# flo-stilz/Audio-Key-Estimation

Measured on AMD Instinct MI355X. Metric: clips/s (15 s @ 22.05 kHz), HIP CQT + PitchClassNet forward, higher is better.
Workload: dtype f32 accumulation everywhere; pitch / semitone / layer-0 convolutions: f16 activations x f16 weights (per-channel power-of-two scaled) on MFMA, one product; last layer's pitch-class convolutions and heads: 3-term split-bf16 on MFMA (hi*hi + lo*hi + hi*lo); CQT filter bank: 3-term split-bf16 on MFMA

## Files before the change

audio-key-estimation_amd/csrc/pcnet_forward.h:

```cpp
#pragma once

namespace {

struct Fwd {
    const ake_pcnet* n;
    Buffers& b;
    hipStream_t s;
    bool train;
    const Route& r;

    float* p2pin_up(int i) const { return train ? b.aff_p2pin[i] + 3 * n->dims[i].prev_p : nullptr; }
    double* stats_of(int bn) const { return b.stats + 2 * n->bns[bn].ch_off; }
    int stats_stride() const { return 2 * n->bn_channels; }

    int finalize_bn(int bn, double count, float* aff_out, float slope = kSlope) {
        const auto& l = n->bns[bn];
        return ake::launch("bn_finalize_kernel", bn_finalize_kernel, dim3((l.C + 63) / 64), dim3(64), 0, s, stats_of(bn), stats_stride(),
                           count, n->blob_dev + l.gamma_off, n->blob_dev + l.beta_off, aff_out, b.bstats + 3 * l.ch_off, l.C, slope);
    }
    int identity(float* aff, int C) {
        return ake::launch_untimed("affine_identity_kernel", affine_identity_kernel, dim3((C + 63) / 64), dim3(64), 0, s, aff, C);
    }

    int conv(const ConvSite& cs, int kind, Src src, const float* in_aff, int B, int H, int T_in, bool same, float* dst, int ctot, int coff,
// ... 368 lines not shown
                    else if (g.in == P2pIn::SrcF16x4)
                        io.src = Src{reinterpret_cast<const float*>(b.melh + static_cast<size_t>(c0) * P * Ti), 1,
                                     reinterpret_cast<const float*>(reinterpret_cast<const uint2*>(b.psix[1]) + static_cast<size_t>(c0) * 36 * Ti), d.prev_pc, 36};
                    else io.src = sdesc;
                    switch (g.out) {
                        case P2pOut::Plane: io.plane = reinterpret_cast<unsigned short*>(out.p); break;
                        case P2pOut::Nchw: io.dst = out.p; break;
                        case P2pOut::Semi: io.dst = out.p; io.semi = &n->semi[i].eval; break;
                        case P2pOut::SemiFold: io.dst = cat; io.dst_ctot = ctot; io.fold_coff = d.prev_pc; io.semi = &n->semi[i].eval; break;
                    }
                    if (last_conv) last_out = g.out;
                    AKE_REQUIRE(g.ok || g.in == P2pIn::Planes || g.in == P2pIn::Src, AKE_ERR_STATE,
                                "pcnet: the route promised an input form only the persistent pitch conv reads, for a chunk (%d clips) it does not take", B);
                    if (g.ok) rc = run_p2p_f16_ps(n, n->p2p[i][j].eval, g, io, B, P, Ti, s, "conv_p2p_f16_kernel");
                    else rc = run_p2p_f16(n, n->p2p[i][j].eval, io.planes, j == 0 ? &io.src : nullptr, B, P, Ti, io.dst, d.out_p, io.plane, s, "conv_p2p_f16_kernel");
                    if (rc) return rc;
                }
            } else if ((rc = stack(0, i, sdesc, in_aff, B, P, Ti, "conv_mfma_kernel/p2p", &out, rp.x3_convs, rk.x3))) return rc;
            if (last_out == P2pOut::SemiFold) {
            } else if (last_out == P2pOut::Semi) {
                if ((rc = run_fold_max("fold_max_kernel", out.p, nullptr, d.out_p, P / 3, B, Ti, cat, ctot, d.prev_pc, s))) return rc;
            } else if (c.stay_sixth && train) {
                if ((rc = run_fold_max("fold_affine_kernel", out.p, out.aff, d.out_p, P, B, Ti, cat, ctot, d.prev_pc, s))) return rc;
                if ((rc = identity(b.aff_cat[i] + 3 * d.prev_pc, d.out_p))) return rc;
            } else if (c.stay_sixth) {
                if ((rc = fold_maps(i, out.p, d.out_p, P, B, Ti, cat, ctot, d.prev_pc))) return rc;
            } else if ((rc = semi(i, out.p, out.aff, B, P, Ti, cat, ctot, d.prev_pc, train ? b.aff_cat[i] + 3 * d.prev_pc : nullptr))) return rc;
            if (last) return AKE_OK;
            Slot pdst;
            if ((rc = stack(1, i, Src{cat, ctot, nullptr, 0, 0}, b.cat_slot(train, i).aff, B, 12, Ti, "conv_mfma_kernel/pc2pc", &pdst))) return rc;
            float* catn = b.cat_at(i + 1, c0);
            if ((rc = time_pool(pdst.p, pdst.aff, B, d.out_pc, 12, Ti, catn, b.cat_ch(i + 1), 0))) return rc;
            if (train && (rc = identity(b.aff_cat[i + 1], d.out_pc))) return rc;
            if ((rc = time_pool(out.p, out.aff, B, d.out_p, P, Ti, b.ppool[i], d.out_p, 0))) return rc;
            pc_cur = catn; p_cur = b.ppool[i]; cp = d.out_p;
        }
        return AKE_OK;
    }

    int last_pc_stack(int B, Slot* feat) {
        const auto& c = n->cfg;
        const int L = c.num_layers, i = L - 1, Ti = b.Tl[i];
        const Slot src = L == 1 ? Slot{b.fold0, nullptr} : b.cat_slot(train, i);
        const int cin = L == 1 ? 1 : n->dims[i].prev_pc + n->dims[i].out_p;
        const char* const label = L == 1 ? "conv_mfma_kernel/pc2pc0" : "conv_mfma_kernel/pc2pc";
        int rc;
        *feat = Slot{b.pcf, nullptr};
        if (r.pc == PcStack::Fused)
            return run_pc2pc_fused(n, i, src.p, cin, B, Ti, b.pcf, r.heads != HeadForm::Generic ? b.feat_cl : nullptr, s);
        Slot out;
        if (r.pc == PcStack::Bf16) {
            const unsigned short* in = reinterpret_cast<const unsigned short*>(b.pcb[i]);
            if ((rc = run_nchw_to_cl16(src.p, cin, B, Ti, reinterpret_cast<unsigned short*>(b.pcb[i]), s))) return rc;
            for (int j = 0; j < c.conv_layers; ++j) {
                const bool last_conv = j == c.conv_layers - 1;
                out = b.pc_out(false, i, j);
                if ((rc = run_pc_bf16(n, n->pc2pc[i][j].eval, in, B, Ti, true, true, last_conv ? out.p : nullptr,
                                      last_conv ? nullptr : reinterpret_cast<unsigned short*>(out.p), s, "conv_pc_bf16_kernel/pc2pc")))
                    return rc;
                in = reinterpret_cast<const unsigned short*>(out.p);
            }
        } else if (c.denseblock) {
            if ((rc = dense_stack(i, 1, src.p, n->final_ch, cin, B, 12, Ti, b.pca[i], label))) return rc;
            out = Slot{src.p, nullptr};
        } else if ((rc = stack(1, i, Src{src.p, cin, nullptr, 0, 0}, src.aff, B, 12, Ti, label, &out, r.pc_x3_convs))) return rc;
        if (L == 1) { *feat = out; return AKE_OK; }
        return time_pool(out.p, out.aff, B, n->final_ch, 12, Ti, b.pcf, n->final_ch, 0);
    }

    int heads_fused(int B, const PoolArgs& pool, float* const outs[3], int* Tm, int* pooled) {
        const int nh = r.genre_bf ? 3 : 2, Tf = b.Tf;
        float* const maps[3] = {b.map_k, b.map_t, b.map_g};
        HeadsFusedArgs ha;
        std::memset(&ha, 0, sizeof(ha));
        ha.xh = b.feat_cl; ha.xl = b.feat_cl + static_cast<long long>(B) * 12 * Tf * 16;
        for (int h = 0; h < nh; ++h) {
            const PackedConv& p0 = n->heads[h].convs[0].eval;
            const PackedConv& p1 = n->heads[h].convs[1].eval;
            ha.bfragA[h] = n->bf_frags_dev + p0.bf_off; ha.biasA[h] = n->blob_dev + p0.b_off; ha.KHA[h] = p0.kh;
            ha.bfragB[h] = n->bf_frags_dev + p1.bf_off; ha.biasB[h] = n->blob_dev + p1.b_off; ha.KHB[h] = p1.kh;
            ha.dst[h] = maps[h];
            ha.pout[h] = outs[h];
        }
        if (r.genre_bf) { ha.hs[0] = 2; ha.hs[1] = 0; ha.hs[2] = 1; }
        else { ha.hs[0] = 0; ha.hs[1] = 1; ha.hs[2] = 1; }
        ha.batch = B; ha.T_in = Tf; ha.T1 = r.T1; ha.T2 = r.T2; ha.TpA = r.T1 + 8; ha.TpB = r.TpB; ha.JB = (r.T2 + 15) / 16;
        ha.fin_off = static_cast<int>(r.hf_lds / sizeof(float)) - 12 * r.T2;
        ha.pool = pool;
        *Tm = r.T2; *pooled = nh;
        static ake::DeviceOnce hf_attr;
        const int rc = ake::raise_lds_limit(hf_attr, 150 * 1024, heads_fused_kernel<3>, heads_fused_kernel<4>);
        if (rc) return rc;
        return r.heads_mt == 3 ? ake::launch("heads_fused_kernel", heads_fused_kernel<3>, dim3(nh * B), dim3(512), r.hf_lds, s, ha)
                               : ake::launch("heads_fused_kernel", heads_fused_kernel<4>, dim3(nh * B), dim3(512), r.hf_lds, s, ha);
    }

    int heads_head1(int B, const PoolArgs& pool, float* const outs[3], int* Tm, int* pooled) {
        const int nh = r.genre_bf ? 3 : 2, Tf = b.Tf, T1 = r.T1, T2 = r.T2;
        const Head* const heads = n->heads;
        float* const maps[3] = {b.map_k, b.map_t, b.map_g};
        Head1BfArgs ha;
        std::memset(&ha, 0, sizeof(ha));
        int rc;
        for (int h = 0; h < nh; ++h) {
            const PackedConv& p0 = heads[h].convs[0].eval;
            const PackedConv& p1 = heads[h].convs[1].eval;
            unsigned short* planes = reinterpret_cast<unsigned short*>(b.head_out(false, h, 0, false).p);
            if (h == 0) {
                PcBf16Opts tonic;
                tonic.pc2 = &heads[1].convs[0].eval; tonic.planes_out2 = reinterpret_cast<unsigned short*>(b.head_out(false, 1, 0, false).p);
                if ((rc = run_pc_bf16(n, p0, b.feat_cl, B, Tf, false, true, nullptr, planes, s, "conv_pc_bf16_kernel/head", tonic))) return rc;
            }
            if (h == 2 && (rc = run_pc_bf16(n, p0, b.feat_cl, B, Tf, false, true, nullptr, planes, s, "conv_pc_bf16_kernel/genre_head")))
                return rc;
            ha.xh[h] = planes; ha.xl[h] = planes + static_cast<long long>(B) * 12 * T1 * 32;
            ha.bfrag[h] = n->bf_frags_dev + p1.bf_off; ha.bias[h] = n->blob_dev + p1.b_off; ha.dst[h] = maps[h];
            ha.KH[h] = p1.kh; ha.circular[h] = p1.kh == 12 ? 1 : 0; ha.H_out[h] = ha.circular[h] ? 12 : 12 - p1.kh + 1;
        }
        ha.T_in = T1; ha.T_out = T2; ha.JB = (T2 + 15) / 16; ha.Tp = r.TpB;
        size_t lds = std::max(static_cast<size_t>(2) * 12 * ha.Tp * 4 * sizeof(uint4), static_cast<size_t>(8) * kHead1MT * 4 * 64 * sizeof(float));
        if (r.heads_pool) {
            ha.fin_off = static_cast<int>(lds / sizeof(float));
            lds += static_cast<size_t>(12) * T2 * sizeof(float);
            for (int h = 0; h < nh; ++h) ha.pout[h] = outs[h];
            ha.pool = pool;
        }
        *Tm = T2; *pooled = r.heads_pool ? nh : 0;
        static ake::DeviceOnce h1_attr;
        if ((rc = ake::raise_lds_limit(h1_attr, 150 * 1024, conv_head1_bf16_kernel))) return rc;
        AKE_REQUIRE(lds <= 150 * 1024, AKE_ERR_UNSUPPORTED, "heads: %d frames do not fit conv_head1_bf16_kernel", T1);
        return ake::launch("conv_head1_bf16_kernel", conv_head1_bf16_kernel, dim3(B, nh), dim3(512), lds, s, ha);
    }

    int heads_generic(int first, Slot feat, int B, int* Tm) {
        const auto& c = n->cfg;
        const Head* const heads = n->heads;
        const int Tf = b.Tf;
        bool head_planes_ready = false;
        int rc;
        for (int h = first; h < (c.genre ? 3 : 2); ++h) {
            for (int j = 0; j < c.head_layers; ++j) {
                const ConvSite& cs = heads[h].convs[j];
                const PackedConv& pe = cs.eval;
                const bool lastj = j == c.head_layers - 1;
                const Slot src = j == 0 ? feat : b.head_out(train, h, j - 1, false);
                const int hc = j == 0 ? n->final_ch : heads[h].convs[j - 1].eval.cout, Tcur = Tf - j * (c.kernel_size - 1);
                const Slot dst = b.head_out(train, h, j, lastj);
                if (r.heads != HeadForm::Generic && h < 2 && j == 0) {
                    if ((rc = run_pc_bf16(n, pe, b.feat_cl, B, Tcur, false, true, dst.p, nullptr, s, "conv_pc_bf16_kernel/head"))) return rc;
                    continue;
                }
                if (train && j == 0 && !lastj && pc_f16x3_ok(cs.train, Tcur, false)) {
                    if (!head_planes_ready) {
                        if ((rc = run_nchw_to_cl16_f16x2(src.p, hc, B, Tcur, src.aff, b.feat_cl, s))) return rc;
                        head_planes_ready = true;
                    }
                    if ((rc = pc_x3_train(cs, b.feat_cl, B, Tcur, false, heads[h].kind == 2 ? 12 - cs.train.kh + 1 : 12, dst,
                                          h == 2 ? "conv_pc_f16x3_kernel/genre_head" : "conv_pc_f16x3_kernel/head")))
                        return rc;
                    continue;
                }
                if (train && lastj && j > 0 && pe.cout == 1 && pe.kw == 7 && !n->raw_w_off.empty()) {
                    const size_t lds = (static_cast<size_t>(hc) * 12 * Tcur + static_cast<size_t>(hc) * pe.kh * 7) * sizeof(float);
                    if (lds <= 150 * 1024 && Tcur - 6 >= 1) {
                        static ake::DeviceOnce hl_attr;
                        if ((rc = ake::raise_lds_limit(hl_attr, 150 * 1024, conv_head_last_kernel))) return rc;
                        if ((rc = ake::launch(h == 2 ? "conv_head_last_kernel/genre" : "conv_head_last_kernel", conv_head_last_kernel, dim3(B), dim3(384), lds, s,
                                              src.p, src.aff, n->blob_dev + n->raw_w_off[cs.w], n->blob_dev + n->raw_w_off[cs.b], dst.p, hc, pe.kh,
                                              heads[h].kind == 2 ? 0 : 1, Tcur, Tcur - 6)))
                            return rc;
                        continue;
                    }
                }
                if ((rc = conv(cs, heads[h].kind, Src{src.p, hc, nullptr, 0, 0}, src.aff, B, 12, Tcur, false, dst.p, pe.cout, 0, dst.aff,
                               h == 2 ? "conv_mfma_kernel/genre_head" : "conv_mfma_kernel/head")))
                    return rc;
            }
// ... 78 lines not shown
```

audio-key-estimation_amd/csrc/pcnet_kernels.h:

```cpp
#pragma once

#include <hip/hip_runtime.h>

#include "bf16_split.h"
#include "common.h"

namespace ake_k {

constexpr int TW = 4;
constexpr float kSlope = 0.01f;

struct ConvArgs {
    const float* src0;
    const float* src1;
    long long src0_clip_stride, src1_clip_stride;
    int c0, c1, h1;
    int H;
    int T_in;
    int T_out;
    int H_out;
    int py;
    int pad_l;
    int time_circ;
    const float* w;
// ... 1625 lines not shown
                            __builtin_amdgcn_sched_barrier(0);
#pragma unroll
                            for (int mt = kFree; mt < MT; ++mt) acc[mt] = __builtin_amdgcn_mfma_f32_16x16x32_bf16(fh[(mt + i) & 3], bl, acc[mt], 0, 0, 0);
#pragma unroll
                            for (int u = 0; u < kFree; ++u) {
                                bw[i + u][0] = wn[((i + u) * 2 + 0) * 64];
                                bw[i + u][1] = wn[((i + u) * 2 + 1) * 64];
                            }
                        }
                    }
                    if (!PAIR || dq < 2) {
                        __builtin_amdgcn_s_waitcnt(0x0F70);
                        asm volatile("s_barrier" ::: "memory");
                    }
                }
            };
#pragma unroll 1
            for (int p = 0; p < 3; ++p) run_p(std::false_type{}, p);
            run_p(std::true_type{}, 3);
            if (active) {
            const int co = r16;
            const float bias = bias_j[co];
            const int tq0 = t0 + 4 * q;
            if (tq0 < T) {
                int e = ((y0 * Tp + tq0 + 3) << 4) + co;
                int g = (co * 12 + y0) * Tf + (tq0 >> 1);
                int ec = (y0 * Tf + (tq0 >> 1)) * 16 + co;
#pragma unroll
                for (int mt = 0; mt < MT; ++mt, e += Tp * 16, g += Tf, ec += Tf * 16) {
                    float v[4];
#pragma unroll
                    for (int i = 0; i < 4; ++i) {
                        const float x = acc[mt][i] + bias;
                        v[i] = x > 0.f ? x : x * kSlope;
                    }
                    if (!last) {
#pragma unroll
                        for (int i = 0; i < 4; i += 2) {
                            unsigned int hi, lo;
                            bf16_split2(v[i], v[i + 1], hi, lo);
                            oH[e + 16 * i] = static_cast<unsigned short>(hi);
                            oH[e + 16 * i + 16] = static_cast<unsigned short>(hi >> 16);
                            oL[e + 16 * i] = static_cast<unsigned short>(lo);
                            oL[e + 16 * i + 16] = static_cast<unsigned short>(lo >> 16);
                        }
                    } else {
                        const float pv0 = fmaxf(v[0], v[1]), pv1 = fmaxf(v[2], v[3]);
                        pooled_c[g] = pv0;
                        pooled_c[g + 1] = pv1;
                        if (a.fh) {
                            unsigned int hi, lo;
                            bf16_split2(pv0, pv1, hi, lo);
                            fh_c[ec] = static_cast<unsigned short>(hi);
                            fh_c[ec + 16] = static_cast<unsigned short>(hi >> 16);
                            fl_c[ec] = static_cast<unsigned short>(lo);
                            fl_c[ec + 16] = static_cast<unsigned short>(lo >> 16);
                        }
                    }
                }
            }
            }
        }
        if (!last) __builtin_amdgcn_s_waitcnt(0x0F70);
        __syncthreads();
    }
}

struct Head1BfArgs {
    const unsigned short* xh[3];
    const unsigned short* xl[3];
    const uint4* bfrag[3];
    const float* bias[3];
    float* dst[3];
    int KH[3], H_out[3], circular[3];
    int T_in, T_out, Tp, JB;
    float* pout[3];
    PoolArgs pool;
    int fin_off;
};

constexpr int kHead1MT = 4;
constexpr int kHead1JB = 5;
__host__ __device__ constexpr int head1_ksteps(int KH) { return KH == 12 ? 12 * 7 : KH * 22; }
constexpr int kHead1PF = 3;

__device__ __forceinline__ void head1_prefetch(const uint4* __restrict__ bg, int nks, int wave, uint4 (&nbh)[kHead1PF], uint4 (&nbl)[kHead1PF]) {
#pragma unroll
    for (int i = 0; i < kHead1PF; ++i) {
        const int kn = wave + 8 * i < nks ? wave + 8 * i : wave;
        nbh[i] = bg[(2 * kn + 0) * 64]; nbl[i] = bg[(2 * kn + 1) * 64];
    }
}

__device__ __forceinline__ void head1_multiply_store(const uint4* __restrict__ bg, int nks, uint4 (&nbh)[kHead1PF], uint4 (&nbl)[kHead1PF], uint4* lds4,
                                                     int Tp, int HO, int circ, int JB, int T_out, int clip, const float* bias_p, float* dst,
                                                     bool keep, int fin_off) {
    constexpr int PF = kHead1PF;
    const int lane = threadIdx.x & 63;
    const int wave = __builtin_amdgcn_readfirstlane(threadIdx.x >> 6);
    const int r16 = lane & 15, q = lane >> 4;
    const uint4* const pH = lds4;
    const uint4* const pL = lds4 + 12 * Tp * 4;
    float* const red = reinterpret_cast<float*>(lds4);
    if (circ) {
        f32x4c acc[kHead1JB];
#pragma unroll
        for (int mt = 0; mt < kHead1JB; ++mt) acc[mt] = f32x4c{0.f, 0.f, 0.f, 0.f};
        for (int ks = wave; ks < nks; ks += 8) {
            const int r = ks / 7, dx = ks - r * 7;
            const bf16x8c bh = __builtin_bit_cast(bf16x8c, nbh[0]);
            const bf16x8c bl = __builtin_bit_cast(bf16x8c, nbl[0]);
#pragma unroll
            for (int i = 0; i + 1 < PF; ++i) { nbh[i] = nbh[i + 1]; nbl[i] = nbl[i + 1]; }
            {
                const int kn = ks + 8 * PF < nks ? ks + 8 * PF : ks;
                nbh[PF - 1] = bg[(2 * kn + 0) * 64]; nbl[PF - 1] = bg[(2 * kn + 1) * 64];
            }
            const int ad0 = ((r * Tp + r16 + dx) << 2) + q;
#pragma unroll
            for (int mt = 0; mt < kHead1JB; ++mt) {
                if (mt < JB) {
                    const bf16x8c ah = __builtin_bit_cast(bf16x8c, pH[ad0 + 64 * mt]);
                    const bf16x8c al = __builtin_bit_cast(bf16x8c, pL[ad0 + 64 * mt]);
                    acc[mt] = __builtin_amdgcn_mfma_f32_16x16x32_bf16(ah, bh, acc[mt], 0, 0, 0);
                    acc[mt] = __builtin_amdgcn_mfma_f32_16x16x32_bf16(al, bh, acc[mt], 0, 0, 0);
                    acc[mt] = __builtin_amdgcn_mfma_f32_16x16x32_bf16(ah, bl, acc[mt], 0, 0, 0);
                }
            }
        }
        __syncthreads();
#pragma unroll
        for (int mt = 0; mt < kHead1JB; ++mt)
            if (mt < JB)
#pragma unroll
                for (int i = 0; i < 4; ++i) red[((wave * JB + mt) * 4 + i) * 64 + lane] = acc[mt][i];
        __syncthreads();
        if (wave < JB) {
            const float bias = bias_p[0];
#pragma unroll
            for (int i = 0; i < 4; ++i) {
                float v = bias;
#pragma unroll
                for (int w = 0; w < 8; ++w) v += red[((w * JB + wave) * 4 + i) * 64 + lane];
                const int t = 16 * wave + 4 * q + i;
                if (r16 < 12 && t < T_out) {
                    dst[(static_cast<long long>(clip) * 12 + r16) * T_out + t] = v;
                    if (keep) red[fin_off + r16 * T_out + t] = v;
                }
            }
        }
        return;
    }
    const int Mtot = HO * JB;
    const int mtiles = (Mtot + 15) / 16;
    int ay[kHead1MT], af[kHead1MT];
#pragma unroll
    for (int mt = 0; mt < kHead1MT; ++mt) {
        int m = mt * 16 + r16;
        if (m >= Mtot) m = Mtot - 1;
        const int jb = m / HO;
        ay[mt] = m - jb * HO;
        af[mt] = 16 * jb;
    }
    f32x4c acc[kHead1MT];
#pragma unroll
    for (int mt = 0; mt < kHead1MT; ++mt) acc[mt] = f32x4c{0.f, 0.f, 0.f, 0.f};
    for (int ks = wave; ks < nks; ks += 8) {
        const int dy = ks / 22, dxe = ks - dy * 22;
        const bf16x8c bh = __builtin_bit_cast(bf16x8c, nbh[0]);
        const bf16x8c bl = __builtin_bit_cast(bf16x8c, nbl[0]);
#pragma unroll
        for (int i = 0; i + 1 < PF; ++i) { nbh[i] = nbh[i + 1]; nbl[i] = nbl[i + 1]; }
        {
            const int kn = ks + 8 * PF < nks ? ks + 8 * PF : ks;
            nbh[PF - 1] = bg[(2 * kn + 0) * 64]; nbl[PF - 1] = bg[(2 * kn + 1) * 64];
        }
#pragma unroll
        for (int mt = 0; mt < kHead1MT; ++mt) {
            if (mt < mtiles) {
                const int ad = (((ay[mt] + dy) * Tp + af[mt] + dxe) << 2) + q;
                const bf16x8c ah = __builtin_bit_cast(bf16x8c, pH[ad]);
                const bf16x8c al = __builtin_bit_cast(bf16x8c, pL[ad]);
                acc[mt] = __builtin_amdgcn_mfma_f32_16x16x32_bf16(ah, bh, acc[mt], 0, 0, 0);
                acc[mt] = __builtin_amdgcn_mfma_f32_16x16x32_bf16(al, bh, acc[mt], 0, 0, 0);
                acc[mt] = __builtin_amdgcn_mfma_f32_16x16x32_bf16(ah, bl, acc[mt], 0, 0, 0);
            }
        }
    }
    __syncthreads();
#pragma unroll
    for (int mt = 0; mt < kHead1MT; ++mt)
#pragma unroll
        for (int i = 0; i < 4; ++i) red[((wave * kHead1MT + mt) * 4 + i) * 64 + lane] = acc[mt][i];
    __syncthreads();
    if (wave < mtiles) {
        const float bias = bias_p[0];
#pragma unroll
        for (int i = 0; i < 4; ++i) {
            float v = bias;
#pragma unroll
            for (int w = 0; w < 8; ++w) v += red[((w * kHead1MT + wave) * 4 + i) * 64 + lane];
            const int m = wave * 16 + 4 * q + i;
            const int jb = m / HO, y = m - jb * HO;
            const int t = 16 * jb + r16;
            if (m < Mtot && t < T_out) {
                dst[(static_cast<long long>(clip) * HO + y) * T_out + t] = v;
                if (keep) red[fin_off + y * T_out + t] = v;
            }
        }
    }
}

__global__ __launch_bounds__(512) void conv_head1_bf16_kernel(Head1BfArgs a) {
    extern __shared__ __attribute__((aligned(16))) uint4 lds4[];
    const int clip = blockIdx.x, head = blockIdx.y;
    const int lane = threadIdx.x & 63;
    const int wave = __builtin_amdgcn_readfirstlane(threadIdx.x >> 6);
    const int Tp = a.Tp;
    uint4* const pH = lds4;
    uint4* const pL = lds4 + 12 * Tp * 4;
    {
        const long long cbase = static_cast<long long>(clip) * 12 * a.T_in * 4;
        const uint4* gh = reinterpret_cast<const uint4*>(a.xh[head]) + cbase;
        const uint4* gl = reinterpret_cast<const uint4*>(a.xl[head]) + cbase;
        const int n16 = 12 * Tp * 4;
        for (int i = threadIdx.x; i < n16; i += blockDim.x) {
            const int grp = i & 3, pos = i >> 2;
            const int row = pos / Tp, f = pos - row * Tp;
            uint4 vh = make_uint4(0, 0, 0, 0), vl = make_uint4(0, 0, 0, 0);
            if (f < a.T_in) {
                const long long g = (static_cast<long long>(row) * a.T_in + f) * 4 + grp;
                vh = gh[g]; vl = gl[g];
            }
            pH[i] = vh; pL[i] = vl;
        }
    }
    __syncthreads();
    const int HO = a.H_out[head], nks = head1_ksteps(a.KH[head]);
    const uint4* __restrict__ bg = a.bfrag[head] + lane;
    uint4 nbh[kHead1PF], nbl[kHead1PF];
    head1_prefetch(bg, nks, wave, nbh, nbl);
    head1_multiply_store(bg, nks, nbh, nbl, lds4, Tp, HO, a.circular[head], a.JB, a.T_out, clip, a.bias[head], a.dst[head], a.pout[head] != nullptr,
                         a.fin_off);
    if (a.pout[head] == nullptr) return;
    __syncthreads();
    if (threadIdx.x < HO)
        a.pout[head][clip * HO + threadIdx.x] =
            pool_row(a.pool, reinterpret_cast<const float*>(lds4) + a.fin_off + threadIdx.x * a.T_out, clip, a.T_out, head);
}

struct HeadsFusedArgs {
    const unsigned short* xh;
    const unsigned short* xl;
    const uint4* bfragA[3];
    const float* biasA[3];
    const uint4* bfragB[3];
    const float* biasB[3];
    float* dst[3];
    float* pout[3];
    int KHA[3], KHB[3];
    int hs[3];
    int batch;
    int T_in, T1, T2;
    int TpA, TpB, JB;
    PoolArgs pool;
    int fin_off;
};

template <int MT>
__global__ __launch_bounds__(512, 4) void heads_fused_kernel(HeadsFusedArgs a) {
    extern __shared__ __attribute__((aligned(16))) uint4 lds4[];
#define AKE_HSEL(f) (head == 0 ? a.f[0] : head == 1 ? a.f[1] : a.f[2])
    const int bid = __builtin_amdgcn_readfirstlane(blockIdx.x);
    const int seg = (bid >= a.batch ? 1 : 0) + (bid >= 2 * a.batch ? 1 : 0);
    const int clip = bid - seg * a.batch;
    const int head = seg == 0 ? a.hs[0] : seg == 1 ? a.hs[1] : a.hs[2];
    const int lane = threadIdx.x & 63;
    const int wave = __builtin_amdgcn_readfirstlane(threadIdx.x >> 6);
    const int r16 = lane & 15, q = lane >> 4;
    constexpr int NT = 2;
    const int TpB = a.TpB;
    uint4* const pHB = lds4;
    uint4* const pLB = lds4 + 12 * TpB * 4;
    const uint4* __restrict__ bg = AKE_HSEL(bfragB) + lane;
    const int KHB = AKE_HSEL(KHB);
    const int nks = head1_ksteps(KHB);
    uint4 nbh[kHead1PF], nbl[kHead1PF];
    {
        const int Mtot = 12 * a.T1;
        const int tile0 = wave * MT;
        const bool active = tile0 * 16 < Mtot;
        f32x4c acc[MT][NT], accl[1][1];
        pc_bf16_multiply<NT, MT, false>(a.xh, a.xl, AKE_HSEL(bfragA), lds4, clip, a.T_in, a.T1, 0, a.TpA, AKE_HSEL(KHA), 8, tile0, Mtot, acc, accl);
        head1_prefetch(bg, nks, wave, nbh, nbl);
        __syncthreads();
        unsigned short* const sH = reinterpret_cast<unsigned short*>(pHB);
        unsigned short* const sL = reinterpret_cast<unsigned short*>(pLB);
        {
            const int nz = TpB - a.T1, n16 = 12 * nz * 4;
            for (int i = threadIdx.x; i < n16; i += 512) {
                const int grp = i & 3, pos = i >> 2;
                const int row = pos / nz, f = a.T1 + pos - row * nz;
                pHB[((row * TpB + f) << 2) + grp] = make_uint4(0, 0, 0, 0);
                pLB[((row * TpB + f) << 2) + grp] = make_uint4(0, 0, 0, 0);
            }
        }
        if (active) {
            const float* const bptr = AKE_HSEL(biasA);
#pragma unroll
            for (int nt = 0; nt < NT; ++nt) {
                const int co = nt * 16 + r16;
                const float bias = bptr[co];
#pragma unroll
                for (int mt = 0; mt < MT; ++mt) {
                    const int m0 = (tile0 + mt) * 16 + 4 * q;
                    int y = m0 / a.T1, t = m0 - y * a.T1;
#pragma unroll
                    for (int i = 0; i < 4; ++i) {
                        if (m0 + i < Mtot) {
                            float v = acc[mt][nt][i] + bias;
                            v = v > 0.f ? v : v * kSlope;
                            const int idx = (y * TpB + t) * 32 + co;
                            const unsigned int hb = bf16_bits(v);
                            sH[idx] = static_cast<unsigned short>(hb);
                            sL[idx] = static_cast<unsigned short>(bf16_bits(v - __uint_as_float(hb << 16)));
                        }
                        if (++t == a.T1) { t = 0; ++y; }
                    }
                }
            }
        }
    }
    __syncthreads();
    const int circ = KHB == 12 ? 1 : 0;
    const int HO = circ ? 12 : 12 - KHB + 1;
    head1_multiply_store(bg, nks, nbh, nbl, lds4, TpB, HO, circ, a.JB, a.T2, clip, AKE_HSEL(biasB), AKE_HSEL(dst), true, a.fin_off);
    __syncthreads();
    if (threadIdx.x < HO)
        AKE_HSEL(pout)[clip * HO + threadIdx.x] = pool_row(a.pool, reinterpret_cast<const float*>(lds4) + a.fin_off + threadIdx.x * a.T2, clip, a.T2, head);
#undef AKE_HSEL
}

__global__ void pack_head1_bf16_kernel(const float* __restrict__ w, uint4* __restrict__ out, int cin, int KH) {
    const int i = blockIdx.x * blockDim.x + threadIdx.x;
    if (i >= head1_ksteps(KH) * 64) return;
    const int lane = i & 63, ks = i >> 6;
    const int col = lane & 15, qq = lane >> 4;
    int dy, dx;
    if (KH == 12) {
        const int r = ks / 7;
        dx = col < 12 ? ks - r * 7 : -1;
        dy = r - col + (r < col ? 12 : 0);
    } else {
        dy = ks / 22;
        dx = ks - dy * 22 - col;
    }
    unsigned int hi[4] = {0, 0, 0, 0}, lo[4] = {0, 0, 0, 0};
    for (int e = 0; e < 8; ++e) {
        const int ci = 8 * qq + e;
        float v = 0.f;
        if (dx >= 0 && dx < 7 && ci < cin) v = w[(ci * KH + dy) * 7 + dx];
        const unsigned int hb = bf16_bits(v);
        hi[e >> 1] |= hb << (16 * (e & 1));
        lo[e >> 1] |= bf16_bits(v - __uint_as_float(hb << 16)) << (16 * (e & 1));
    }
    out[(2 * ks + 0) * 64 + lane] = make_uint4(hi[0], hi[1], hi[2], hi[3]);
    out[(2 * ks + 1) * 64 + lane] = make_uint4(lo[0], lo[1], lo[2], lo[3]);
}

__global__ void pack_pc_bf16_kernel(const float* __restrict__ w, uint4* __restrict__ out, int cin, int cout, int CO, int NT, int KH) {
    const int i = blockIdx.x * blockDim.x + threadIdx.x;
    if (i >= KH * 4 * NT * 64) return;
    const int lane = i & 63, nt = (i >> 6) % NT, ks = i / (64 * NT);
    const int dy = ks >> 2, p = ks & 3;
    const int co = nt * 16 + (lane & 15), qq = lane >> 4;
    const int c8 = 8 * (qq & 1);
    int dx = 2 * p + (qq >> 1), dyw = dy;
    if (p == 3 && !(KH & 1)) {
        dx = (dy & 1) ? 7 : 6;
        dyw = dy + (qq >> 1);
    }
    unsigned int hi[4] = {0, 0, 0, 0}, lo[4] = {0, 0, 0, 0};
    for (int e = 0; e < 8; ++e) {
        const int ci = c8 + e;
        float v = 0.f;
        if (dx < 7 && ci < cin && co < cout) v = w[((((co / CO) * cin + ci) * KH + dyw) * 7 + dx) * CO + (co % CO)];
        const unsigned int hb = bf16_bits(v);
        const unsigned int lb = bf16_bits(v - __uint_as_float(hb << 16));
        hi[e >> 1] |= hb << (16 * (e & 1));
        lo[e >> 1] |= lb << (16 * (e & 1));
    }
    out[((ks * NT + nt) * 2 + 0) * 64 + lane] = make_uint4(hi[0], hi[1], hi[2], hi[3]);
    out[((ks * NT + nt) * 2 + 1) * 64 + lane] = make_uint4(lo[0], lo[1], lo[2], lo[3]);
}

__global__ void nchw_to_cl16_kernel(const float* __restrict__ src, long long src_clip_stride, int C, int T, unsigned short* __restrict__ xh,
                                    unsigned short* __restrict__ xl, long long npos) {
    const long long i = static_cast<long long>(blockIdx.x) * blockDim.x + threadIdx.x;
    if (i >= npos) return;
    const int t = static_cast<int>(i % T);
    const long long r = i / T;
    const int y = static_cast<int>(r % 12);
    const long long clip = r / 12;
    const float* s = src + clip * src_clip_stride + static_cast<long long>(y) * T + t;
    unsigned int hi[8], lo[8];
#pragma unroll
    for (int k = 0; k < 8; ++k) { hi[k] = 0; lo[k] = 0; }
#pragma unroll
    for (int c = 0; c < 16; ++c) {
        const float v = c < C ? s[static_cast<long long>(c) * 12 * T] : 0.f;
        const unsigned int hb = bf16_bits(v);
        hi[c >> 1] |= hb << (16 * (c & 1));
        lo[c >> 1] |= bf16_bits(v - __uint_as_float(hb << 16)) << (16 * (c & 1));
    }
    uint4* oh = reinterpret_cast<uint4*>(xh) + i * 2;
    uint4* ol = reinterpret_cast<uint4*>(xl) + i * 2;
    oh[0] = make_uint4(hi[0], hi[1], hi[2], hi[3]); oh[1] = make_uint4(hi[4], hi[5], hi[6], hi[7]);
    ol[0] = make_uint4(lo[0], lo[1], lo[2], lo[3]); ol[1] = make_uint4(lo[4], lo[5], lo[6], lo[7]);
}

__global__ void nchw_to_cl16_f16x2_kernel(const float* __restrict__ src, long long src_clip_stride, int C, int T, const float* __restrict__ aff,
                                          unsigned short* __restrict__ xh, unsigned short* __restrict__ xl, long long npos,
                                          const unsigned int* __restrict__ amax) {
// ... 980 lines not shown
```

audio-key-estimation_amd/csrc/pcnet_plan.h:

```cpp
#pragma once

namespace {

struct Slot {
    float* p = nullptr;
    float* aff = nullptr;
};

struct Buffers {
    float* fold0 = nullptr;
    unsigned int* melh = nullptr;
    float* smap = nullptr;
    float* p0 = nullptr;
    std::vector<float*> pcd;
    std::vector<float*> cat, psix, pa, pb, pca, pcb, ppool, pin;
    float *pcf = nullptr, *hid_k = nullptr, *hid_t = nullptr, *hid_g = nullptr;
    float *map_k = nullptr, *map_t = nullptr, *map_g = nullptr;
    size_t hid_half = 0;
    std::vector<int> Tl;
    int Tf = 0;
    size_t bytes = 0;
    double* stats = nullptr;
    float* bstats = nullptr;
    std::vector<float*> semi_raw, aff_semi, aff_cat, aff_p2pin;
// ... 241 lines not shown
Route build_route(const ake_pcnet* n, bool train, int batch, int chunk, int frames, const float* mel, const void* ws, bool mel_fm) {
    Route r;
    const auto& c = n->cfg;
    const int L = c.num_layers;
    const bool ws16 = !(reinterpret_cast<uintptr_t>(ws) & 15);
    int Tl[4], Tf;
    layer_frames(c, frames, Tl, &Tf);
    if (batch < 1 || chunk < 1 || Tf < 1) return r;
    r.chunk_clips[0] = std::min(batch, chunk);
    r.chunk_clips[1] = batch > chunk ? batch % chunk : 0;

    if (!train && L > 1) r.l0 = layer0_plan(n, Tl[0], !(reinterpret_cast<uintptr_t>(mel) & 15), mel_fm);
    if (r.l0.form == L0Form::FusedMfma && !g_keep_taps && !c.pc2p_mem && n->dims[1].prev_p == 1 && p2p_uses_f16(n, 1, Tl[1])) {
        r.psix_f16 = true;
        for (int k = 0; k < 2 && r.psix_f16; ++k)
            if (r.chunk_clips[k])
                r.psix_f16 = p2p_ps_plan(P2pIn::SrcF16x4, 1, n->dims[1].prev_pc, P2pOut::Plane, n->dims[1].out_p, false, r.chunk_clips[k], c.pitches, Tl[1], ws16).ok;
    }

    const int P = c.stay_sixth ? c.pitches / 3 : c.pitches;
    int cp = 1;
    for (int i = 1; i < L && !c.denseblock && !c.resblock; ++i) {
        const LayerDims& d = n->dims[i];
        Route::Pitch& rp = r.p[i];
        const int Ti = Tl[i], c0 = cp, c1 = c.pc2p_mem ? 0 : d.prev_pc;
        if (!train && p2p_uses_f16(n, i, Ti)) {
            rp.stack = PStack::F16;
            const bool semi = p2p_fuses_semi(n, i, P, Ti);
            for (int k = 0; k < 2; ++k) {
                const int B = r.chunk_clips[k];
                if (!B) continue;
                const P2pIn in0 = (i == 1 && r.psix_f16) ? P2pIn::SrcF16x4 : ((mel_fm && i == 1) ? P2pIn::SrcFramesMajor : P2pIn::Src);
                rp.k[k].first = p2p_ps_plan(in0, c0, c1, P2pOut::Plane, d.out_p, false, B, P, Ti, ws16);
                rp.k[k].mid = p2p_ps_plan(P2pIn::Planes, 0, 0, P2pOut::Plane, d.out_p, false, B, P, Ti, ws16);
                P2pPsPlan& last = rp.k[k].last;
                if (semi) last = p2p_ps_plan(P2pIn::Planes, 0, 0, P2pOut::SemiFold, d.prev_pc + d.out_p, true, B, P, Ti, ws16);
                if (semi && !last.ok) last = p2p_ps_plan(P2pIn::Planes, 0, 0, P2pOut::Semi, d.out_p, true, B, P, Ti, ws16);
                if (!last.ok) last = p2p_ps_plan(P2pIn::Planes, 0, 0, P2pOut::Nchw, d.out_p, false, B, P, Ti, ws16);
                if (in0 == P2pIn::SrcF16x4 && semi) rp.k[k].stack = p2p_stack_plan(c.conv_layers, c0, c1, true, B, P, Ti);
            }
        } else if (!c.pc2p_mem && !c.stay_sixth && (train || (c.precision == AKE_PRECISION_F32X3 && !g_keep_taps))) {
            for (int k = 0; k < 2; ++k) {
                const int B = r.chunk_clips[k];
                if (!B) continue;
                rp.k[k].x3[0] = p2p_f16x3_plan(c0, c1, d.out_p, B, P, Ti, ws16);
                rp.k[k].x3[1] = p2p_f16x3_plan(d.out_p, 0, d.out_p, B, P, Ti, ws16);
            }
            for (int j = 0; j < c.conv_layers && j < 32; ++j)
                if ((train ? n->p2p[i][j].train : n->p2p[i][j].eval).bf_off >= 0 && rp.k[0].x3[j > 0].ok) rp.x3_convs |= 1u << j;
            if (rp.x3_convs) rp.stack = PStack::F16x3;
        }
        cp = d.out_p;
    }
    r.frames_major = mel_fm && !train && L == 2 && !c.resblock && !c.denseblock && !c.pc2p_mem && !c.p2pc_conv && !c.stay_sixth && !c.local &&
                     batch <= chunk && r.l0.form == L0Form::FusedMfma && r.p[1].stack == PStack::F16 && r.p[1].k[0].first.ok;

    const int i = L - 1, Ti = Tl[i];
    if (!train && L > 1 && !c.denseblock && pc2pc_fuses(n, i, Ti)) r.pc = PcStack::Fused;
    else if (!train && pc2pc_uses_bf16(n, i, Ti)) r.pc = PcStack::Bf16;
    else if (train && L > 1 && !c.resblock && !c.denseblock) {
        for (int j = 0; j < c.conv_layers && j < 32; ++j)
            if (pc_f16x3_ok(n->pc2pc[i][j].train, Ti, true)) r.pc_x3_convs |= 1u << j;
        if (r.pc_x3_convs) r.pc = PcStack::F16x3;
    }

    const std::vector<ConvSite>&hk = n->heads[0].convs, &ht = n->heads[1].convs, &hg = n->heads[2].convs;
    const bool head_bf = !train && L > 1 && n->final_ch == 16 && c.head_layers >= 2 && hk[0].eval.bf_off >= 0 && ht[0].eval.bf_off >= 0 &&
                         Tf <= kPcBf16MaxFrames;
    if (!head_bf) return r;
    r.heads = HeadForm::Bf16First;
    r.T1 = Tf - (c.kernel_size - 1); r.T2 = r.T1 - (c.kernel_size - 1);
    const int T1 = r.T1, T2 = r.T2;
    if (!(c.head_layers == 2 && hk[1].eval.bf_off >= 0 && ht[1].eval.bf_off >= 0 && T2 > 0 && (12 * ((T2 + 15) / 16) + 15) / 16 <= kHead1MT)) return r;
    r.heads = HeadForm::Head1;
    r.genre_bf = c.genre && hg.size() == 2 && hg[0].eval.bf_off >= 0 && hg[1].eval.bf_off >= 0 && hg[0].eval.kh == 1 && hg[1].eval.kh == 2;
    r.heads_pool = c.local == 0;
    r.TpB = 16 * ((T2 + 15) / 16 - 1) + 22;
    r.hf_lds = std::max({(static_cast<size_t>(2) * 12 * (T1 + 8) * 2 + 2 * 4 * 2 * 2 * 64) * sizeof(uint4),
                         static_cast<size_t>(2) * 12 * r.TpB * 4 * sizeof(uint4),
                         static_cast<size_t>(8) * kHead1MT * 4 * 64 * sizeof(float)}) +
               static_cast<size_t>(12) * T2 * sizeof(float);
    if (r.pc == PcStack::Fused && !g_keep_taps && c.local == 0 && hk[0].eval.cout == 32 && ht[0].eval.cout == 32 && hk[0].eval.kh == 12 &&
        ht[0].eval.kh == 12 && hk[1].eval.kh == 12 && ht[1].eval.kh == 12 && (!r.genre_bf || hg[0].eval.cout == 32) &&
        (12 * T1 + 15) / 16 <= 32 && r.hf_lds <= 150 * 1024) {
        r.heads = HeadForm::Fused;
        r.heads_mt = (12 * T1 + 15) / 16 <= 24 ? 3 : 4;
    }
    return r;
}

}
```

Before: 492,600.

## Restructure fused heads kernel: genre head run inside key/tonic blocks, deeper weight prefetch

```diff
diff --git a/audio-key-estimation_amd/csrc/pcnet_forward.h b/audio-key-estimation_amd/csrc/pcnet_forward.h
--- a/audio-key-estimation_amd/csrc/pcnet_forward.h
+++ b/audio-key-estimation_amd/csrc/pcnet_forward.h
@@ -474,8 +474,8 @@
             ha.dst[h] = maps[h];
             ha.pout[h] = outs[h];
         }
-        if (r.genre_bf) { ha.hs[0] = 2; ha.hs[1] = 0; ha.hs[2] = 1; }
-        else { ha.hs[0] = 0; ha.hs[1] = 1; ha.hs[2] = 1; }
+        ha.genre_rows = r.genre_bf ? 12 - n->heads[2].convs[1].eval.kh + 1 : 0;
+        ha.genre_split = ha.genre_rows;
         ha.batch = B; ha.T_in = Tf; ha.T1 = r.T1; ha.T2 = r.T2; ha.TpA = r.T1 + 8; ha.TpB = r.TpB; ha.JB = (r.T2 + 15) / 16;
         ha.fin_off = static_cast<int>(r.hf_lds / sizeof(float)) - 12 * r.T2;
         ha.pool = pool;
@@ -483,8 +483,8 @@
         static ake::DeviceOnce hf_attr;
         const int rc = ake::raise_lds_limit(hf_attr, 150 * 1024, heads_fused_kernel<3>, heads_fused_kernel<4>);
         if (rc) return rc;
-        return r.heads_mt == 3 ? ake::launch("heads_fused_kernel", heads_fused_kernel<3>, dim3(nh * B), dim3(512), r.hf_lds, s, ha)
-                               : ake::launch("heads_fused_kernel", heads_fused_kernel<4>, dim3(nh * B), dim3(512), r.hf_lds, s, ha);
+        return r.heads_mt == 3 ? ake::launch("heads_fused_kernel", heads_fused_kernel<3>, dim3(2 * B), dim3(512), r.hf_lds, s, ha)
+                               : ake::launch("heads_fused_kernel", heads_fused_kernel<4>, dim3(2 * B), dim3(512), r.hf_lds, s, ha);
     }
 
     int heads_head1(int B, const PoolArgs& pool, float* const outs[3], int* Tm, int* pooled) {
diff --git a/audio-key-estimation_amd/csrc/pcnet_kernels.h b/audio-key-estimation_amd/csrc/pcnet_kernels.h
--- a/audio-key-estimation_amd/csrc/pcnet_kernels.h
+++ b/audio-key-estimation_amd/csrc/pcnet_kernels.h
@@ -1731,58 +1731,131 @@
 constexpr int kHead1MT = 4;
 constexpr int kHead1JB = 5;
 __host__ __device__ constexpr int head1_ksteps(int KH) { return KH == 12 ? 12 * 7 : KH * 22; }
-constexpr int kHead1PF = 3;
-
+constexpr int kHead1PF = 6;
+
+template <int I0 = 0, int I1 = kHead1PF>
 __device__ __forceinline__ void head1_prefetch(const uint4* __restrict__ bg, int nks, int wave, uint4 (&nbh)[kHead1PF], uint4 (&nbl)[kHead1PF]) {
 #pragma unroll
-    for (int i = 0; i < kHead1PF; ++i) {
+    for (int i = I0; i < I1; ++i) {
         const int kn = wave + 8 * i < nks ? wave + 8 * i : wave;
         nbh[i] = bg[(2 * kn + 0) * 64]; nbl[i] = bg[(2 * kn + 1) * 64];
     }
 }
 
+template <int JB>
+__device__ __forceinline__ void head1_circ_tiles(const uint4* __restrict__ bg, uint4 (&nbh)[kHead1PF], uint4 (&nbl)[kHead1PF], const uint4* pH,
+                                                 const uint4* pL, float* red, int Tp) {
+    constexpr int PF = kHead1PF, NKS = head1_ksteps(12), NS = (NKS + 7) / 8;
+    const int lane = threadIdx.x & 63;
+    const int wave = __builtin_amdgcn_readfirstlane(threadIdx.x >> 6);
+    const int r16 = lane & 15, q = lane >> 4;
+    f32x4c acc[JB];
+#pragma unroll
+    for (int mt = 0; mt < JB; ++mt) acc[mt] = f32x4c{0.f, 0.f, 0.f, 0.f};
+#pragma unroll
+    for (int st = 0; st < NS; ++st) {
+        const int ks = wave + 8 * st;
+        if (8 * st + 7 >= NKS && ks >= NKS) break;
+        const int r = ks / 7, dx = ks - r * 7;
+        const bf16x8c bh = __builtin_bit_cast(bf16x8c, nbh[st % PF]);
+        const bf16x8c bl = __builtin_bit_cast(bf16x8c, nbl[st % PF]);
+        const int ad0 = ((r * Tp + r16 + dx) << 2) + q;
+#pragma unroll
+        for (int mt = 0; mt < JB; ++mt) {
+            const bf16x8c ah = __builtin_bit_cast(bf16x8c, pH[ad0 + 64 * mt]);
+            const bf16x8c al = __builtin_bit_cast(bf16x8c, pL[ad0 + 64 * mt]);
+            acc[mt] = __builtin_amdgcn_mfma_f32_16x16x32_bf16(ah, bh, acc[mt], 0, 0, 0);
+            acc[mt] = __builtin_amdgcn_mfma_f32_16x16x32_bf16(al, bh, acc[mt], 0, 0, 0);
+            acc[mt] = __builtin_amdgcn_mfma_f32_16x16x32_bf16(ah, bl, acc[mt], 0, 0, 0);
+            if (JB > 3 && (mt & 1) && mt + 1 < JB) __builtin_amdgcn_sched_barrier(0);
+        }
+        if (st + PF < NS) {
+            const int kn = ks + 8 * PF < NKS ? ks + 8 * PF : ks;
+            nbh[st % PF] = bg[(2 * kn + 0) * 64]; nbl[st % PF] = bg[(2 * kn + 1) * 64];
+        }
+        __builtin_amdgcn_sched_barrier(0);
+    }
+    __syncthreads();
+#pragma unroll
+    for (int mt = 0; mt < JB; ++mt)
+#pragma unroll
+        for (int i = 0; i < 4; ++i) red[((wave * JB + mt) * 4 + i) * 64 + lane] = acc[mt][i];
+}
+
+template <int J, int JBM>
+__device__ __forceinline__ void head1_circ_pick(int JB, const uint4* __restrict__ bg, uint4 (&nbh)[kHead1PF], uint4 (&nbl)[kHead1PF], const uint4* pH,
+                                                const uint4* pL, float* red, int Tp) {
+    if constexpr (J == JBM) head1_circ_tiles<J>(bg, nbh, nbl, pH, pL, red, Tp);
+    else if (JB <= J) head1_circ_tiles<J>(bg, nbh, nbl, pH, pL, red, Tp);
+    else head1_circ_pick<J + 1, JBM>(JB, bg, nbh, nbl, pH, pL, red, Tp);
+}
+
+template <int NMT>
+__device__ __forceinline__ void head1_valid_tiles(const uint4* __restrict__ bg, int nks, uint4 (&nbh)[kHead1PF], uint4 (&nbl)[kHead1PF], const uint4* pH,
+                                                  const uint4* pL, float* red, int Tp, int JB, int y0, int HOr) {
+    constexpr int PF = kHead1PF;
+    const int lane = threadIdx.x & 63;
+    const int wave = __builtin_amdgcn_readfirstlane(threadIdx.x >> 6);
+    const int r16 = lane & 15, q = lane >> 4;
+    const int Mtot = HOr * JB;
+    const int mtiles = (Mtot + 15) / 16;
+    int ad0[NMT];
+#pragma unroll
+    for (int mt = 0; mt < NMT; ++mt) {
+        int m = mt * 16 + r16;
+        if (m >= Mtot) m = Mtot - 1;
+        const int jb = m / HOr;
+        ad0[mt] = (((y0 + m - jb * HOr) * Tp + 16 * jb) << 2) + q;
+    }
+    f32x4c acc[NMT];
+#pragma unroll
+    for (int mt = 0; mt < NMT; ++mt) acc[mt] = f32x4c{0.f, 0.f, 0.f, 0.f};
+    for (int ks0 = wave; ks0 < nks; ks0 += 8 * PF) {
+        const bool more = ks0 + 8 * PF < nks;
+#pragma unroll
+        for (int j = 0; j < PF; ++j) {
+            const int ks = ks0 + 8 * j;
+            if (ks >= nks) goto done;
+            const int dy = ks / 22, dxe = ks - dy * 22;
+            const bf16x8c bh = __builtin_bit_cast(bf16x8c, nbh[j]);
+            const bf16x8c bl = __builtin_bit_cast(bf16x8c, nbl[j]);
+#pragma unroll
+            for (int mt = 0; mt < NMT; ++mt) {
+                if (mt < mtiles) {
+                    const int ad = ad0[mt] + ((dy * Tp + dxe) << 2);
+                    const bf16x8c ah = __builtin_bit_cast(bf16x8c, pH[ad]);
+                    const bf16x8c al = __builtin_bit_cast(bf16x8c, pL[ad]);
+                    acc[mt] = __builtin_amdgcn_mfma_f32_16x16x32_bf16(ah, bh, acc[mt], 0, 0, 0);
+                    acc[mt] = __builtin_amdgcn_mfma_f32_16x16x32_bf16(al, bh, acc[mt], 0, 0, 0);
+                    acc[mt] = __builtin_amdgcn_mfma_f32_16x16x32_bf16(ah, bl, acc[mt], 0, 0, 0);
+                }
+            }
+            if (more) {
+                const int kn = ks + 8 * PF < nks ? ks + 8 * PF : ks;
+                nbh[j] = bg[(2 * kn + 0) * 64]; nbl[j] = bg[(2 * kn + 1) * 64];
+            }
+        }
+    }
+done:
+    __syncthreads();
+#pragma unroll
+    for (int mt = 0; mt < NMT; ++mt)
+#pragma unroll
+        for (int i = 0; i < 4; ++i) red[((wave * kHead1MT + mt) * 4 + i) * 64 + lane] = acc[mt][i];
+}
+
+template <bool CIRC, int JBM, int MTM>
 __device__ __forceinline__ void head1_multiply_store(const uint4* __restrict__ bg, int nks, uint4 (&nbh)[kHead1PF], uint4 (&nbl)[kHead1PF], uint4* lds4,
-                                                     int Tp, int HO, int circ, int JB, int T_out, int clip, const float* bias_p, float* dst,
-                                                     bool keep, int fin_off) {
-    constexpr int PF = kHead1PF;
+                                                     int Tp, int HO, int JB, int T_out, int clip, const float* bias_p, float* dst,
+                                                     bool keep, int fin_off, int y0, int HOr) {
     const int lane = threadIdx.x & 63;
     const int wave = __builtin_amdgcn_readfirstlane(threadIdx.x >> 6);
     const int r16 = lane & 15, q = lane >> 4;
     const uint4* const pH = lds4;
     const uint4* const pL = lds4 + 12 * Tp * 4;
     float* const red = reinterpret_cast<float*>(lds4);
-    if (circ) {
-        f32x4c acc[kHead1JB];
-#pragma unroll
-        for (int mt = 0; mt < kHead1JB; ++mt) acc[mt] = f32x4c{0.f, 0.f, 0.f, 0.f};
-        for (int ks = wave; ks < nks; ks += 8) {
-            const int r = ks / 7, dx = ks - r * 7;
-            const bf16x8c bh = __builtin_bit_cast(bf16x8c, nbh[0]);
-            const bf16x8c bl = __builtin_bit_cast(bf16x8c, nbl[0]);
-#pragma unroll
-            for (int i = 0; i + 1 < PF; ++i) { nbh[i] = nbh[i + 1]; nbl[i] = nbl[i + 1]; }
-            {
-                const int kn = ks + 8 * PF < nks ? ks + 8 * PF : ks;
-                nbh[PF - 1] = bg[(2 * kn + 0) * 64]; nbl[PF - 1] = bg[(2 * kn + 1) * 64];
-            }
-            const int ad0 = ((r * Tp + r16 + dx) << 2) + q;
-#pragma unroll
-            for (int mt = 0; mt < kHead1JB; ++mt) {
-                if (mt < JB) {
-                    const bf16x8c ah = __builtin_bit_cast(bf16x8c, pH[ad0 + 64 * mt]);
-                    const bf16x8c al = __builtin_bit_cast(bf16x8c, pL[ad0 + 64 * mt]);
-                    acc[mt] = __builtin_amdgcn_mfma_f32_16x16x32_bf16(ah, bh, acc[mt], 0, 0, 0);
-                    acc[mt] = __builtin_amdgcn_mfma_f32_16x16x32_bf16(al, bh, acc[mt], 0, 0, 0);
-                    acc[mt] = __builtin_amdgcn_mfma_f32_16x16x32_bf16(ah, bl, acc[mt], 0, 0, 0);
-                }
-            }
-        }
-        __syncthreads();
-#pragma unroll
-        for (int mt = 0; mt < kHead1JB; ++mt)
-            if (mt < JB)
-#pragma unroll
-                for (int i = 0; i < 4; ++i) red[((wave * JB + mt) * 4 + i) * 64 + lane] = acc[mt][i];
+    if (CIRC) {
+        head1_circ_pick<1, JBM>(JB, bg, nbh, nbl, pH, pL, red, Tp);
         __syncthreads();
         if (wave < JB) {
             const float bias = bias_p[0];
@@ -1800,47 +1873,9 @@
         }
         return;
     }
-    const int Mtot = HO * JB;
+    const int Mtot = HOr * JB;
     const int mtiles = (Mtot + 15) / 16;
-    int ay[kHead1MT], af[kHead1MT];
-#pragma unroll
-    for (int mt = 0; mt < kHead1MT; ++mt) {
-        int m = mt * 16 + r16;
-        if (m >= Mtot) m = Mtot - 1;
-        const int jb = m / HO;
-        ay[mt] = m - jb * HO;
-        af[mt] = 16 * jb;
-    }
-    f32x4c acc[kHead1MT];
-#pragma unroll
-    for (int mt = 0; mt < kHead1MT; ++mt) acc[mt] = f32x4c{0.f, 0.f, 0.f, 0.f};
-    for (int ks = wave; ks < nks; ks += 8) {
-        const int dy = ks / 22, dxe = ks - dy * 22;
-        const bf16x8c bh = __builtin_bit_cast(bf16x8c, nbh[0]);
-        const bf16x8c bl = __builtin_bit_cast(bf16x8c, nbl[0]);
-#pragma unroll
-        for (int i = 0; i + 1 < PF; ++i) { nbh[i] = nbh[i + 1]; nbl[i] = nbl[i + 1]; }
-        {
-            const int kn = ks + 8 * PF < nks ? ks + 8 * PF : ks;
-            nbh[PF - 1] = bg[(2 * kn + 0) * 64]; nbl[PF - 1] = bg[(2 * kn + 1) * 64];
-        }
-#pragma unroll
-        for (int mt = 0; mt < kHead1MT; ++mt) {
-            if (mt < mtiles) {
-                const int ad = (((ay[mt] + dy) * Tp + af[mt] + dxe) << 2) + q;
-                const bf16x8c ah = __builtin_bit_cast(bf16x8c, pH[ad]);
-                const bf16x8c al = __builtin_bit_cast(bf16x8c, pL[ad]);
-                acc[mt] = __builtin_amdgcn_mfma_f32_16x16x32_bf16(ah, bh, acc[mt], 0, 0, 0);
-                acc[mt] = __builtin_amdgcn_mfma_f32_16x16x32_bf16(al, bh, acc[mt], 0, 0, 0);
-                acc[mt] = __builtin_amdgcn_mfma_f32_16x16x32_bf16(ah, bl, acc[mt], 0, 0, 0);
-            }
-        }
-    }
-    __syncthreads();
-#pragma unroll
-    for (int mt = 0; mt < kHead1MT; ++mt)
-#pragma unroll
-        for (int i = 0; i < 4; ++i) red[((wave * kHead1MT + mt) * 4 + i) * 64 + lane] = acc[mt][i];
+    head1_valid_tiles<MTM>(bg, nks, nbh, nbl, pH, pL, red, Tp, JB, y0, HOr);
     __syncthreads();
     if (wave < mtiles) {
         const float bias = bias_p[0];
@@ -1850,7 +1885,7 @@
 #pragma unroll
             for (int w = 0; w < 8; ++w) v += red[((w * kHead1MT + wave) * 4 + i) * 64 + lane];
             const int m = wave * 16 + 4 * q + i;
-            const int jb = m / HO, y = m - jb * HO;
+            const int jb = m / HOr, y = y0 + m - jb * HOr;
             const int t = 16 * jb + r16;
             if (m < Mtot && t < T_out) {
                 dst[(static_cast<long long>(clip) * HO + y) * T_out + t] = v;
@@ -1887,10 +1922,17 @@
     __syncthreads();
     const int HO = a.H_out[head], nks = head1_ksteps(a.KH[head]);
     const uint4* __restrict__ bg = a.bfrag[head] + lane;
-    uint4 nbh[kHead1PF], nbl[kHead1PF];
-    head1_prefetch(bg, nks, wave, nbh, nbl);
-    head1_multiply_store(bg, nks, nbh, nbl, lds4, Tp, HO, a.circular[head], a.JB, a.T_out, clip, a.bias[head], a.dst[head], a.pout[head] != nullptr,
-                         a.fin_off);
+    if (a.circular[head]) {
+        uint4 nbh[kHead1PF], nbl[kHead1PF];
+        head1_prefetch(bg, nks, wave, nbh, nbl);
+        head1_multiply_store<true, kHead1JB, kHead1MT>(bg, nks, nbh, nbl, lds4, Tp, HO, a.JB, a.T_out, clip, a.bias[head], a.dst[head],
+                                                       a.pout[head] != nullptr, a.fin_off, 0, HO);
+    } else {
+        uint4 nbh[kHead1PF], nbl[kHead1PF];
+        head1_prefetch(bg, nks, wave, nbh, nbl);
+        head1_multiply_store<false, kHead1JB, kHead1MT>(bg, nks, nbh, nbl, lds4, Tp, HO, a.JB, a.T_out, clip, a.bias[head], a.dst[head],
+                                                        a.pout[head] != nullptr, a.fin_off, 0, HO);
+    }
     if (a.pout[head] == nullptr) return;
     __syncthreads();
     if (threadIdx.x < HO)
@@ -1908,86 +1950,117 @@
     float* dst[3];
     float* pout[3];
     int KHA[3], KHB[3];
-    int hs[3];
     int batch;
+    int genre_rows;
+    int genre_split;
     int T_in, T1, T2;
     int TpA, TpB, JB;
     PoolArgs pool;
     int fin_off;
 };
 
-template <int MT>
-__global__ __launch_bounds__(512, 4) void heads_fused_kernel(HeadsFusedArgs a) {
-    extern __shared__ __attribute__((aligned(16))) uint4 lds4[];
+constexpr int kHeadsFusedJB = 3, kHeadsFusedMT = 2;
+
+template <int MT, bool CIRC>
+__device__ __forceinline__ void heads_fused_pass(const HeadsFusedArgs& a, uint4* lds4, int clip, int head, int y0, int HOr) {
 #define AKE_HSEL(f) (head == 0 ? a.f[0] : head == 1 ? a.f[1] : a.f[2])
-    const int bid = __builtin_amdgcn_readfirstlane(blockIdx.x);
-    const int seg = (bid >= a.batch ? 1 : 0) + (bid >= 2 * a.batch ? 1 : 0);
-    const int clip = bid - seg * a.batch;
-    const int head = seg == 0 ? a.hs[0] : seg == 1 ? a.hs[1] : a.hs[2];
     const int lane = threadIdx.x & 63;
     const int wave = __builtin_amdgcn_readfirstlane(threadIdx.x >> 6);
     const int r16 = lane & 15, q = lane >> 4;
     constexpr int NT = 2;
-    const int TpB = a.TpB;
+    const int T1 = a.T1, TpB = a.TpB;
     uint4* const pHB = lds4;
     uint4* const pLB = lds4 + 12 * TpB * 4;
     const uint4* __restrict__ bg = AKE_HSEL(bfragB) + lane;
     const int KHB = AKE_HSEL(KHB);
     const int nks = head1_ksteps(KHB);
+    const int HO = CIRC ? 12 : 12 - KHB + 1;
+    const int h0 = CIRC ? 0 : y0, h1 = CIRC ? 12 : y0 + HOr + KHB - 1;
     uint4 nbh[kHead1PF], nbl[kHead1PF];
     {
-        const int Mtot = 12 * a.T1;
-        const int tile0 = wave * MT;
-        const bool active = tile0 * 16 < Mtot;
+        const int Mend = h1 * T1;
+        const int tile0 = (h0 * T1) / 16 + wave * MT;
+        const bool active = tile0 * 16 < Mend;
         f32x4c acc[MT][NT], accl[1][1];
-        pc_bf16_multiply<NT, MT, false>(a.xh, a.xl, AKE_HSEL(bfragA), lds4, clip, a.T_in, a.T1, 0, a.TpA, AKE_HSEL(KHA), 8, tile0, Mtot, acc, accl);
-        head1_prefetch(bg, nks, wave, nbh, nbl);
+        pc_bf16_multiply<NT, MT, false>(a.xh, a.xl, AKE_HSEL(bfragA), lds4, clip, a.T_in, T1, 0, a.TpA, AKE_HSEL(KHA), 8, tile0, Mend, acc, accl);
+        const float* const bptr = AKE_HSEL(biasA);
+        const float bias0 = bptr[r16], bias1 = bptr[16 + r16];
+        head1_prefetch<0, kHead1PF / 2>(bg, nks, wave, nbh, nbl);
+        __builtin_amdgcn_sched_barrier(0);
         __syncthreads();
         unsigned short* const sH = reinterpret_cast<unsigned short*>(pHB);
         unsigned short* const sL = reinterpret_cast<unsigned short*>(pLB);
         {
-            const int nz = TpB - a.T1, n16 = 12 * nz * 4;
+            const int nz = TpB - T1, n16 = (h1 - h0) * nz * 4;
             for (int i = threadIdx.x; i < n16; i += 512) {
                 const int grp = i & 3, pos = i >> 2;
-                const int row = pos / nz, f = a.T1 + pos - row * nz;
-                pHB[((row * TpB + f) << 2) + grp] = make_uint4(0, 0, 0, 0);
-                pLB[((row * TpB + f) << 2) + grp] = make_uint4(0, 0, 0, 0);
+                const int row = pos / nz, f = T1 + pos - row * nz;
+                pHB[(((h0 + row) * TpB + f) << 2) + grp] = make_uint4(0, 0, 0, 0);
+                pLB[(((h0 + row) * TpB + f) << 2) + grp] = make_uint4(0, 0, 0, 0);
             }
         }
         if (active) {
-            const float* const bptr = AKE_HSEL(biasA);
-#pragma unroll
-            for (int nt = 0; nt < NT; ++nt) {
-                const int co = nt * 16 + r16;
-                const float bias = bptr[co];
-#pragma unroll
-                for (int mt = 0; mt < MT; ++mt) {
-                    const int m0 = (tile0 + mt) * 16 + 4 * q;
-                    int y = m0 / a.T1, t = m0 - y * a.T1;
-#pragma unroll
-                    for (int i = 0; i < 4; ++i) {
-                        if (m0 + i < Mtot) {
-                            float v = acc[mt][nt][i] + bias;
-                            v = v > 0.f ? v : v * kSlope;
-                            const int idx = (y * TpB + t) * 32 + co;
-                            const unsigned int hb = bf16_bits(v);
-                            sH[idx] = static_cast<unsigned short>(hb);
-                            sL[idx] = static_cast<unsigned short>(bf16_bits(v - __uint_as_float(hb << 16)));
+            int m = tile0 * 16 + 4 * q;
+            const int y = m / T1;
+            int t = m - y * T1;
+            int idx = (y * TpB + t) * 32 + r16;
+            const int wrap = (TpB - T1) * 32;
+#pragma unroll
+            for (int mt = 0; mt < MT; ++mt) {
+#pragma unroll
+                for (int i = 0; i < 4; i += 2) {
+                    float v[NT][2];
+#pragma unroll
+                    for (int nt = 0; nt < NT; ++nt)
+#pragma unroll
+                        for (int e = 0; e < 2; ++e) {
+                            const float x = acc[mt][nt][i + e] + (nt == 0 ? bias0 : bias1);
+                            v[nt][e] = x > 0.f ? x : x * kSlope;
                         }
-                        if (++t == a.T1) { t = 0; ++y; }
+                    unsigned int hi[NT], lo[NT];
+#pragma unroll
+                    for (int nt = 0; nt < NT; ++nt) bf16_split2(v[nt][0], v[nt][1], hi[nt], lo[nt]);
+#pragma unroll
+                    for (int e = 0; e < 2; ++e) {
+                        if (m < Mend) {
+#pragma unroll
+                            for (int nt = 0; nt < NT; ++nt) {
+                                sH[idx + 16 * nt] = static_cast<unsigned short>(hi[nt] >> (16 * e));
+                                sL[idx + 16 * nt] = static_cast<unsigned short>(lo[nt] >> (16 * e));
+                            }
+                        }
+                        ++m; idx += 32;
+                        if (++t == T1) { t = 0; idx += wrap; }
                     }
                 }
-            }
-        }
+                m += 12; t += 12; idx += 12 * 32;
+                if (t >= T1) { t -= T1; idx += wrap; }
+                if (t >= T1) { t -= T1; idx += wrap; }
+            }
+        }
+        head1_prefetch<kHead1PF / 2, kHead1PF>(bg, nks, wave, nbh, nbl);
+        __builtin_amdgcn_sched_barrier(0);
     }
     __syncthreads();
-    const int circ = KHB == 12 ? 1 : 0;
-    const int HO = circ ? 12 : 12 - KHB + 1;
-    head1_multiply_store(bg, nks, nbh, nbl, lds4, TpB, HO, circ, a.JB, a.T2, clip, AKE_HSEL(biasB), AKE_HSEL(dst), true, a.fin_off);
+    head1_multiply_store<CIRC, kHeadsFusedJB, kHeadsFusedMT>(bg, nks, nbh, nbl, lds4, TpB, HO, a.JB, a.T2, clip, AKE_HSEL(biasB), AKE_HSEL(dst), true, a.fin_off, y0, HOr);
     __syncthreads();
-    if (threadIdx.x < HO)
+    if (static_cast<int>(threadIdx.x) >= y0 && static_cast<int>(threadIdx.x) < y0 + HOr)
         AKE_HSEL(pout)[clip * HO + threadIdx.x] = pool_row(a.pool, reinterpret_cast<const float*>(lds4) + a.fin_off + threadIdx.x * a.T2, clip, a.T2, head);
 #undef AKE_HSEL
+}
+
+template <int MT>
+__global__ __launch_bounds__(512, 4) void heads_fused_kernel(HeadsFusedArgs a) {
+    extern __shared__ __attribute__((aligned(16))) uint4 lds4[];
+    const int bid = __builtin_amdgcn_readfirstlane(blockIdx.x);
+    const int head = bid >= a.batch ? 1 : 0;
+    const int clip = bid - head * a.batch;
+    heads_fused_pass<MT, true>(a, lds4, clip, head, 0, 12);
+    if (!a.genre_rows) return;
+    __syncthreads();
+    const int gy0 = head == 0 ? 0 : a.genre_split, gn = head == 0 ? a.genre_split : a.genre_rows - a.genre_split;
+    if (gn <= 0) return;
+    heads_fused_pass<MT, false>(a, lds4, clip, 2, gy0, gn);
 }
 
 __global__ void pack_head1_bf16_kernel(const float* __restrict__ w, uint4* __restrict__ out, int cin, int KH) {
diff --git a/audio-key-estimation_amd/csrc/pcnet_plan.h b/audio-key-estimation_amd/csrc/pcnet_plan.h
--- a/audio-key-estimation_amd/csrc/pcnet_plan.h
+++ b/audio-key-estimation_amd/csrc/pcnet_plan.h
@@ -347,7 +347,8 @@
                static_cast<size_t>(12) * T2 * sizeof(float);
     if (r.pc == PcStack::Fused && !g_keep_taps && c.local == 0 && hk[0].eval.cout == 32 && ht[0].eval.cout == 32 && hk[0].eval.kh == 12 &&
         ht[0].eval.kh == 12 && hk[1].eval.kh == 12 && ht[1].eval.kh == 12 && (!r.genre_bf || hg[0].eval.cout == 32) &&
-        (12 * T1 + 15) / 16 <= 32 && r.hf_lds <= 150 * 1024) {
+        (12 * T1 + 15) / 16 <= 32 && r.hf_lds <= 150 * 1024 &&
+        (T2 + 15) / 16 <= kHeadsFusedJB && (!r.genre_bf || ((12 - hg[1].eval.kh + 1) * ((T2 + 15) / 16) + 15) / 16 <= kHeadsFusedMT)) {
         r.heads = HeadForm::Fused;
         r.heads_mt = (12 * T1 + 15) / 16 <= 24 ? 3 : 4;
     }
```

New measurement: 492,500. Within noise of the previous version (-0.0%).
